# dglai/dgl-0.5-benchmark

Hardware: AMD Instinct MI355X
Metric: aggregated edges/s, full-graph 3-layer GraphSAGE (hidden 64) on an ogbn-products-shaped graph; epoch time in ms_per_step (higher is better)
Workload: dtype f32

## Files before the change

### dgl-0.5-benchmark_amd/csrc/xty.hip

```cpp
#include "common.h"

namespace mgx {

constexpr int kXtyWaves = 2048;

static int xty_waves(int64_t n) {
  int64_t w = (n / 256 + 63) / 64 * 64;
  if (w < 256) w = 256;
  if (w > kXtyWaves) w = kXtyWaves;
  return (int)w;
}

template <int MT, int KT>
__global__ __launch_bounds__(kBlock) void xty_partial_kernel(int64_t n, int M, int K, const float* __restrict__ A, int64_t lda,
                                                             const float* __restrict__ B, int64_t ldb, float* __restrict__ part) {
  const int lane = threadIdx.x & (kWave - 1);
  const int64_t gw = (int64_t)blockIdx.x * kWavesPerBlock + threadIdx.x / kWave;
  const int c = lane % 16, q = lane / 16;
  v4f acc[MT][KT];
#pragma unroll
  for (int i = 0; i < MT; ++i)
#pragma unroll
    for (int j = 0; j < KT; ++j) acc[i][j] = (v4f)(0.f);
  bool am[MT], bm[KT];
// ... 272 lines not shown
  __syncthreads();
  if (sl == 0 && live) {
    float s = 0.f;
    for (int i = 0; i < 16; ++i) s += red[i][e];
    out[(int64_t)(m0 + m) * ldc + k0 + k] = s;
  }
}

template <int MT>
static bool launch_xty_kt(int kt, int waves, int64_t n, int M, int K, const float* A, int64_t lda, const float* B, int64_t ldb,
                          float* part, hipStream_t s) {
  switch (kt) {
#define MGX_XTY(J) case J: hipLaunchKernelGGL((xty_partial_kernel<MT, J>), dim3(waves / kWavesPerBlock), dim3(kBlock), 0, s, n, M, K, A, lda, B, ldb, part); return true;
    MGX_XTY(1) MGX_XTY(2) MGX_XTY(3) MGX_XTY(4) MGX_XTY(5) MGX_XTY(6) MGX_XTY(7) MGX_XTY(8)
#undef MGX_XTY
    default: return false;
  }
}

}

namespace mgx {
__global__ __launch_bounds__(kBlock) void xty_colsum_finish_kernel(int M, int mt16, int waves, const float* __restrict__ part_sum,
                                                                   float* __restrict__ colsum) {
  const int m = blockIdx.x * kWavesPerBlock + threadIdx.x / kWave;
  const int lane = threadIdx.x % kWave;
  if (m >= M) return;
  float s = 0.f;
  for (int w = lane; w < waves; w += kWave) s += part_sum[(int64_t)w * mt16 + m];
#pragma unroll
  for (int off = 32; off >= 1; off >>= 1) s += __shfl_xor(s, off, kWave);
  if (lane == 0) colsum[m] = s;
}
}

extern "C" int64_t mgx_xty_workspace(int64_t M, int64_t K) {
  const int64_t mt = (M + 15) / 16, kt = (K + 15) / 16;
  if (M < 1 || K < 1) return -1;
  if (mt > 4 || kt > 8) {
    if (M > 256 || K > 1024) return -1;
    return (int64_t)mgx::kXtyGridTotal * mgx::kXtyTileM * mgx::kXtyTileK * (int64_t)sizeof(float);
  }
  return (int64_t)mgx::kXtyWaves * (mt * 16 * kt * 16 + mt * 16) * (int64_t)sizeof(float);
}

static int32_t xty_impl(int64_t n, int64_t M, int64_t K, const float* a, int64_t lda, const float* b, int64_t ldb, float* out, int64_t ldc,
                        float* colsum, void* workspace, void* stream, const int64_t* b_rows = nullptr, int mode = 0);

extern "C" int32_t mgx_xty(int64_t n, int64_t M, int64_t K, const float* a, int64_t lda, const float* b, int64_t ldb, float* out,
                           int64_t ldc, void* workspace, void* stream) {
  return xty_impl(n, M, K, a, lda, b, ldb, out, ldc, nullptr, workspace, stream);
}

extern "C" int32_t mgx_xty_colsum(int64_t n, int64_t M, int64_t K, const float* a, int64_t lda, const float* b, int64_t ldb, float* out,
                                  int64_t ldc, float* colsum, void* workspace, void* stream) {
  if (!colsum) return xty_impl(n, M, K, a, lda, b, ldb, out, ldc, nullptr, workspace, stream);
  return xty_impl(n, M, K, a, lda, b, ldb, out, ldc, colsum, workspace, stream);
}

extern "C" int32_t mgx_xty_rows(int64_t n, int64_t M, int64_t K, const float* a, int64_t lda, const float* b, int64_t ldb,
                                const int64_t* b_rows, float* out, int64_t ldc, void* workspace, void* stream) {
  return xty_impl(n, M, K, a, lda, b, ldb, out, ldc, nullptr, workspace, stream, b_rows, b_rows ? mgx::kXtyBRows : 0);
}

extern "C" int32_t mgx_xty_colsum_rows(int64_t n, int64_t M, int64_t K, const float* a, int64_t lda, const float* b, int64_t ldb,
                                       const int64_t* b_rows, float* out, int64_t ldc, float* colsum, void* workspace, void* stream) {
// ... 33 lines not shown
    if (wpt > by_rows) wpt = (int)by_rows;
    if (wpt < 64) wpt = 64;
    hipLaunchKernelGGL(xty_partial_grid_kernel, dim3(wpt / kWavesPerBlock, tiles_m * tiles_k), dim3(kBlock), 0, s, n, (int)M,
                       (int)K, tiles_k, a, lda, b, ldb, part);
    MGX_CHECK_LAUNCH();
    hipLaunchKernelGGL(xty_finish_grid_kernel, dim3(kXtyTileM * kXtyTileK / 16, tiles_m * tiles_k), dim3(kBlock), 0, s, (int)M, (int)K,
                       tiles_k, wpt, (const float*)part, out, ldc);
    MGX_CHECK_LAUNCH();
    return MGX_OK;
  }
  const int waves = xty_waves(n);
  float* part_sum = colsum ? part + (int64_t)kXtyWaves * mt * 16 * kt * 16 : nullptr;
  bool ok = launch_xty_v4(mt, kt, waves, n, (int)M, (int)K, a, lda, b, ldb, part, part_sum, s, b_rows, mode);
  if (!ok && b_rows) MGX_UNSUPPORTED("mgx_xty_rows: no row-list kernel for %lld x %lld", (long long)M, (long long)K);
  if (!ok && colsum) MGX_UNSUPPORTED("mgx_xty_colsum: needs the 16-byte-load form (B: K %% 4 == 0, K >= 64, aligned)");
  if (!ok) switch (mt) {
    case 1: ok = launch_xty_kt<1>(kt, waves, n, (int)M, (int)K, a, lda, b, ldb, part, s); break;
    case 2: ok = launch_xty_kt<2>(kt, waves, n, (int)M, (int)K, a, lda, b, ldb, part, s); break;
    case 3: ok = launch_xty_kt<3>(kt, waves, n, (int)M, (int)K, a, lda, b, ldb, part, s); break;
    default: ok = launch_xty_kt<4>(kt, waves, n, (int)M, (int)K, a, lda, b, ldb, part, s); break;
  }
  MGX_CHECK_ARG(ok, "mgx_xty: no kernel for this tile shape");
  MGX_CHECK_LAUNCH();
  hipLaunchKernelGGL(xty_finish_kernel, dim3((unsigned)((M * K + 15) / 16)), dim3(kBlock), 0, s, (int)M, (int)K, kt * 16,
                     mt * 16 * kt * 16, waves, (const float*)part, out, ldc);
  MGX_CHECK_LAUNCH();
  if (colsum) {
    hipLaunchKernelGGL(xty_colsum_finish_kernel, dim3((unsigned)((M + kWavesPerBlock - 1) / kWavesPerBlock)), dim3(kBlock), 0, s, (int)M,
                       mt * 16, waves, (const float*)part_sum, colsum);
    MGX_CHECK_LAUNCH();
  }
  return MGX_OK;
}
```

### dgl-0.5-benchmark_amd/mi355x_graph/_lib.py

```python
import ctypes
import os

_HERE = os.path.dirname(os.path.abspath(__file__))
CSRC_DIR = os.path.normpath(os.path.join(_HERE, "..", "csrc"))
LIB_PATH = os.environ.get("MGX_LIB_PATH") or os.path.join(CSRC_DIR, "libmi355x_graph.so")
HEADER_PATH = os.path.normpath(os.path.join(_HERE, "..", "..", "include", "mi355x_graph.h"))


class DGLError(RuntimeError):
    """Error type of the DGL operator surface (re-exported as dgl.DGLError)."""


class MgxCsr(ctypes.Structure):
    _fields_ = [
        ("num_rows", ctypes.c_int64),
        ("num_cols", ctypes.c_int64),
        ("nnz", ctypes.c_int64),
        ("indptr", ctypes.c_void_p),
        ("indices", ctypes.c_void_p),
        ("eids", ctypes.c_void_p),
        ("idx_bits", ctypes.c_int32),
        ("reserved", ctypes.c_int32),
    ]

# ... 53 lines not shown
    "mgx_dot_attention_supported": (_i32, [_csr_p, _i64, _i64]),
    "mgx_dot_attention_workspace": (_i64, [_vp, _i64, _i64]),
    "mgx_dot_attention_fwd": (_i32, [_csr_p, _vp, _i64, _i64, _fp, _i64, _fp, _i64, _fp, _i64, ctypes.c_float, _fp, _fp, _vp, _vp]),
    "mgx_dot_attention_bwd": (_i32, [_csr_p, _vp, _csr_p, _vp, _i64, _i64, _fp, _i64, _fp, _i64, _fp, _i64, ctypes.c_float, _fp, _fp, _fp,
                                     _fp, _fp, _fp, _vp, _vp]),
    "mgx_gine_supported": (_i32, [_csr_p, _i64]),
    "mgx_gine_workspace": (_i64, [_vp, _i64]),
    "mgx_gine_fwd": (_i32, [_csr_p, _vp, _i64, _fp, _fp, _fp, _fp, _vp, _vp]),
    "mgx_gine_bwd": (_i32, [_csr_p, _vp, _i64, _fp, _fp, _fp, _fp, _fp, _fp, _vp, _vp]),
    "mgx_head_dot_fwd": (_i32, [_i64, _i64, _i64, _fp, _fp, _fp, _fp, _fp, _vp]),
    "mgx_head_dot_bwd_workspace": (_i64, [_i64, _i64]),
    "mgx_head_dot_bwd": (_i32, [_i64, _i64, _i64, _fp, _fp, _fp, _fp, _fp, _fp, _fp, _fp, _vp, _vp]),
    "mgx_segment_reduce": (_i32, [_i64, _vp, _i64, _i32, _fp, _fp, _vp, _vp]),
    "mgx_segment_softmax_fwd": (_i32, [_i64, _vp, _i64, _fp, _fp, _vp]),
    "mgx_segment_softmax_bwd": (_i32, [_i64, _vp, _i64, _fp, _fp, _fp, _vp]),
    "mgx_segment_attention_supported": (_i32, [_i64, _i64, _i64]),
    "mgx_segment_attention_fwd": (_i32, [_i64, _vp, _i64, _i64, _fp, _i64, _fp, _fp, ctypes.c_float, _fp, _fp, _vp]),
    "mgx_segment_attention_bwd": (_i32, [_i64, _vp, _i64, _i64, _fp, _i64, _fp, _fp, ctypes.c_float, _fp, _fp, _fp, _fp, _fp, _fp, _vp]),
    "mgx_relu_dropout_fwd": (_i32, [_i64, _fp, ctypes.c_float, ctypes.c_uint64, ctypes.c_uint64, _fp, _vp, _vp]),
    "mgx_relu_dropout_bwd": (_i32, [_i64, _fp, _vp, ctypes.c_float, _fp, _vp]),
    "mgx_relu_dropout_fwd_strided": (_i32, [_i64, _i64, _fp, _i64, ctypes.c_float, ctypes.c_uint64, ctypes.c_uint64, _fp, _i64, _vp, _vp]),
    "mgx_relu_dropout_bwd_strided": (_i32, [_i64, _i64, _fp, _i64, _vp, ctypes.c_float, _fp, _i64, _vp]),
    "mgx_relu_dropout_bwd_slots": (_i32, [_i64, _fp, _i64, _vp, ctypes.c_float, _fp, _i64, _fp, _vp, _vp, _vp]),
    "mgx_relu_dropout_fwd_counter": (_i32, [_i64, _i64, _fp, _i64, ctypes.c_float, ctypes.c_uint64, _vp, _fp, _i64, _vp, _vp]),
    "mgx_column_pair_sums": (_i32, [_i64, _i64, _i32, _fp, _fp, _fp, _fp, _vp, _vp]),
    "mgx_column_affine": (_i32, [_i64, _i64, _fp, _fp, _fp, _fp, _fp, _fp, _vp]),
    "mgx_xty_workspace": (_i64, [_i64, _i64]),
    "mgx_xty": (_i32, [_i64, _i64, _i64, _fp, _i64, _fp, _i64, _fp, _i64, _vp, _vp]),
    "mgx_xty_colsum": (_i32, [_i64, _i64, _i64, _fp, _i64, _fp, _i64, _fp, _i64, _fp, _vp, _vp]),
    "mgx_rows_gemm": (_i32, [_i64, _i64, _i64, _fp, _i64, _fp, _i64, _i32, _fp, _fp, _i64, _fp, _i64, _fp, _i64, _i64, _vp]),
    "mgx_xty_rows": (_i32, [_i64, _i64, _i64, _fp, _i64, _fp, _i64, _vp, _fp, _i64, _vp, _vp]),
    "mgx_xty_colsum_rows": (_i32, [_i64, _i64, _i64, _fp, _i64, _fp, _i64, _vp, _fp, _i64, _fp, _vp, _vp]),
    "mgx_xty_colsum_pos": (_i32, [_i64, _i64, _i64, _fp, _i64, _vp, _fp, _i64, _fp, _i64, _fp, _vp, _vp]),
    "mgx_rows_gemm_rows": (_i32, [_i64, _i64, _i64, _fp, _i64, _vp, _fp, _i64, _i32, _fp, _fp, _i64, _fp, _i64, _fp, _i64, _i64, _vp, _vp]),
    "mgx_rows_gemm_supported": (_i32, [_i64, _i64, _i64]),
    "mgx_rows_gemm_sweep_rows": (_i64, [_i64, _i64, _i64, _i32]),
    "mgx_rows_gemm_relu_dropout": (_i32, [_i64, _i64, _i64, _fp, _i64, _fp, _i64, _i32, _fp, ctypes.c_float, ctypes.c_uint64, ctypes.c_uint64,
                                          _fp, _i64, _vp, _vp, _vp, _vp]),
    "mgx_column_sum_workspace": (_i64, [_i64]),
    "mgx_column_sum": (_i32, [_i64, _i64, _fp, _fp, _vp, _vp]),
    "mgx_coo_to_csr_workspace": (_i64, [_i64, _i64, _i32]),
    "mgx_coo_to_csr": (_i32, [_i64, _i64, _vp, _vp, _i32, _vp, _vp, _vp, _vp, _i64, _vp]),
    "mgx_csr_transpose_workspace": (_i64, [_i64, _i64, _i32]),
    "mgx_csr_transpose": (_i32, [_csr_p, _vp, _vp, _vp, _vp, _i64, _vp]),
    "mgx_csr_degrees": (_i32, [_i64, _vp, _i32, _vp, _vp]),
    "mgx_csr_inv_degrees": (_i32, [_i64, _vp, _i32, _fp, _vp]),
    "mgx_coo_to_csr_host": (_i32, [_i64, _i64, _vp, _vp, _i32, _vp, _vp, _vp]),
    "mgx_sample_neighbors": (_i32, [_csr_p, _i64, _vp, _i32, ctypes.c_uint64, _vp, _vp, _vp, _vp]),
    "mgx_sample_count_positive": (_i32, [_csr_p, _i64, _vp, _fp, _vp, _vp, _vp]),
    "mgx_sample_neighbors_weighted": (_i32, [_csr_p, _i64, _vp, _i32, _fp, _i32, ctypes.c_uint64, _vp, _vp, _vp, _vp]),
    "mgx_select_topk": (_i32, [_csr_p, _i64, _vp, _i32, _fp, _i32, _vp, _vp, _vp, _vp]),
    "mgx_to_block_workspace": (_i64, [_i64, _i64]),
    "mgx_to_block": (_i32, [_i64, _i64, _vp, _i64, _vp, _vp, _i32, _i32, _vp, _vp, _vp, _vp, _vp, _vp, _vp]),
    "mgx_node_subgraph_workspace": (_i64, [_i64]),
    "mgx_node_subgraph_count": (_i32, [_csr_p, _i64, _vp, _vp, _vp, _vp, _vp]),
    "mgx_node_subgraph_fill": (_i32, [_csr_p, _i64, _vp, _vp, _vp, _i32, _vp, _vp, _vp, _vp]),
    "mgx_gather_rows": (_i32, [_i64, _vp, _i32, _i64, _fp, _fp, _vp]),
    "mgx_gather_rows_strided": (_i32, [_i64, _vp, _i32, _i64, _fp, _i64, _fp, _i64, _vp]),
    "mgx_scatter_add_rows": (_i32, [_i64, _vp, _i32, _i64, _fp, _fp, _vp]),
}

_lib = None


def lib():
    global _lib
# ... 22 lines not shown
```

### dgl-0.5-benchmark_amd/mi355x_graph/config.py

```python

SAGE_FUSED_LAYER = True
SAGE_CAT = True
SAGE_STATIC_CAT = True
SAGE_FUSED_ADD = True
SAGE_FUSED_ACT = True
SAGE_PROJECT_FIRST = True
SAGE_HEAD_ROWS = True
SAGE_HEAD_INIT = True
ROWS_GEMM = True
LINEAR_XTY = True
XTY_COLSUM = True

GAT_AGG_FIRST = True
GAT_PACK = True

DOT_ATTENTION_FUSED = True
GINE_FUSED = True

SEGMENT_ATTENTION_FUSED = True

DEVICE_BLOCKS = True
DEVICE_SUBGRAPH = True

PLAN_BUILDER = "device"
HUB_SPLIT = 256
LP_ROUNDS = 8
CLUSTER_MIN_NNZ = 4_000_000
TILE_HUB_SPLIT = 2048
TILE_CONFIG = {4: (7, 6, 1, 3), 3: (7, 3, 1, 3), 2: (7, 3, 1, 2)}
GAT_TILE_CONFIG = (7, 3, 1, 2)
TILE_MIN_WIDTH = 4
TILE_VALIDATE = True
SHORT_ROWS_IMBALANCE = 6.0

SPARSE_GRAD = False
SPARSE_GRAD_MIN_NNZ = 2_000_000
WIDE_PAD = True
WIDE_PAD_MIN_NNZ = 1 << 20

PACKED_GATHER = True
PACKED_GATHER_MIN_NNZ = 20_000_000
PACKED_GATHER_PROBE = True
PACKED_GATHER_MAX_OVERFLOW = 0.10

# ... 3 lines not shown
```

### dgl-0.5-benchmark_amd/mi355x_graph/dist.py

```python
import os

import torch
from torch.autograd.function import once_differentiable
import torch.distributed as dist
import torch.nn as nn

from ._lib import DGLError
from . import core, emulate, ops, schedule, sparse
from . import config
from . import function as fn
from .graph import DGLGraph, Frame, GraphIndex


def partition_nodes(src, dst, num_nodes, num_parts, rounds=5, clusters=None):
    dev = src.device
    if num_parts == 1:
        return torch.zeros(num_nodes, dtype=torch.int64, device=dev), {"edge_cut": 0.0, "num_clusters": 1}
    indeg = torch.bincount(dst.long(), minlength=num_nodes)
    node_w = indeg + 1
    if clusters is None:
        csc = sparse.coo_to_csr(num_nodes, num_nodes, dst.contiguous(), src.contiguous())
        cap = int(node_w.sum().item()) // (num_parts * 4) + 1
        hist = schedule.label_propagation(csc.indptr, csc.indices, num_nodes, rounds)
        clusters = _cap_clusters(hist, node_w, cap)
# ... 498 lines not shown
        if plan.n_halo:
            be.spmm_copy_u_strided(plan.halo.csc(), "sum", recv, cat.right, accumulate=True, dst_scale=plan.inv_deg)
        ctx.plan, ctx.comm, ctx.cat, ctx.generation = plan, comm, cat, cat.generation
        ctx.halo_x = halo_x
        comm.mark("dense")
        wcat = torch.cat([w_self, w_neigh], dim=1)
        if act is not None:
            p, into = act
            seed = torch.initial_seed() & (2 ** 64 - 1)
            offset = (ops.ReluDropout._calls * 0x9E3779B97F4A7C15) & (2 ** 63 - 1)
            ops.ReluDropout._calls += 1
            out = None if into is None else into.t
            fused = be.rows_gemm_relu_dropout(cat.buf, wcat, True, bias, float(p), seed, offset, out=out)
            y, mask = fused if fused is not None else be.relu_dropout_fwd(ops._rows_linear(be, cat.buf, wcat, bias), float(p), seed, offset, out=out)
            ctx.save_for_backward(w_self, w_neigh, mask)
            ctx.p = float(p)
            return y
        ctx.save_for_backward(w_self, w_neigh)
        ctx.p = None
        return ops._rows_linear(be, cat.buf, wcat, bias)

    @staticmethod
    @once_differentiable
    def backward(ctx, dy):
        from . import ops
        plan, comm, cat = ctx.plan, ctx.comm, ctx.cat
        if cat.generation != ctx.generation:
            raise DGLError("SAGEConv: a later forward pass overwrote the [h | neigh] buffer this backward pass needs")
        be = sparse.backend_for(dy)
        if ctx.p is not None:
            w_self, w_neigh, mask = ctx.saved_tensors
            if not dy.is_contiguous() and not (hasattr(be, "_row_strided") and be._row_strided(dy)):
                dy = dy.contiguous()
            dy = be.relu_dropout_bwd(dy, mask, ctx.p)
        else:
            w_self, w_neigh = ctx.saved_tensors
        dy = dy.contiguous()
        need = ctx.needs_input_grad
        K = cat.K
        dh = None
        if need[3]:
            dh_own, dn = ops._rows_dgrad(be, dy, torch.cat([w_self, w_neigh], dim=1), plan.inv_deg, K)
            halo_x = ctx.halo_x
            g_halo = torch.empty((plan.n_halo, K), dtype=dy.dtype, device=dy.device)
            comm.mark("halo-row gradients")
            if plan.n_halo:
                be.spmm_copy_u_strided(plan.halo.csr(), "sum", dn, g_halo)
            if halo_x is not None:
                comm.mark("pack")
                halo_x.post_back(g_halo)
            else:
                back = torch.empty((plan.send_idx.shape[0], K), dtype=dy.dtype, device=dy.device)
                work = comm.all_to_all_async(back, g_halo, plan.send_splits, plan.recv_splits)
            comm.mark("owned-row reversed aggregation")
            be.spmm_copy_u_strided(plan.loc.csr(), "sum", dn, dh_own, accumulate=True)
        comm.mark("dense (inside the exchange window)")
        dws = dwn = db = None
        if (need[4] or need[5]) and need[6]:
            dw, db = ops._weight_bias_grad(dy, cat.buf)
            dws, dwn = dw[:, :K].contiguous(), dw[:, K:].contiguous()
        elif need[4] or need[5]:
            dw = ops._weight_grad(dy, cat.buf)
            dws, dwn = dw[:, :K].contiguous(), dw[:, K:].contiguous()
        elif need[6]:
            db = be.column_sum(dy)
        if need[3]:
# ... 447 lines not shown
```

### dgl-0.5-benchmark_amd/mi355x_graph/ops.py

```python
import os

import torch
from torch.autograd.function import once_differentiable

from ._lib import DGLError
from . import sparse
from . import config
from .graph import DGLGraph, GraphIndex

__all__ = ["gspmm", "rel_gspmm", "gsddmm", "edge_softmax", "gat_attention", "gat_fused", "dot_attention", "dot_attention_fused", "gine_sum", "gine_sum_fused", "segment_reduce", "segment_softmax", "segment_attention", "segment_attention_fused", "copy_u_sum", "copy_u_mean", "u_mul_e_sum",
           "copy_e_sum", "u_add_v", "u_dot_v"]


def _torch_ops():
    if os.environ.get("MGX_TORCH_OPS", "auto") != "1":
        return None
    from . import torch_ops
    return torch_ops


_NATIVE = None


def _native_ops():
# ... 761 lines not shown
        n = x.shape[0]
        sdy, sdyx = be.column_pair_sums(dy, x, shifted=True)
        sdyxhat = (sdyx - (mean - x[0]) * sdy) * invstd
        A = invstd if weight is None else weight * invstd
        B = -A * invstd * sdyxhat / n
        Cc = -A * sdy / n - B * mean
        dx = be.column_affine(dy, A.contiguous(), Cc.contiguous(), x, B.contiguous()) if ctx.needs_input_grad[0] else None
        dw = sdyxhat if weight is not None and ctx.needs_input_grad[1] else None
        db = sdy if ctx.needs_input_grad[2] else None
        return dx, dw, db, None


def batch_norm_supported(x):
    return (x.dim() == 2 and x.dtype == torch.float32 and x.device.type in sparse._BACKENDS and x.shape[1] % 4 == 0
            and 4 <= x.shape[1] <= sparse.backend_for(x).COLUMN_SUM_MAX and x.shape[0] > 1)


def _weight_grad(dy2, x2):
    be = sparse.backend_for(dy2)
    if (x2.shape[0] >= be.XTY_MIN_ROWS and dy2.shape[1] <= be.XTY_MAX[0] and x2.shape[1] <= be.XTY_MAX[1]
            and config.LINEAR_XTY):
        return be.xty(dy2 if dy2.stride(1) == 1 else dy2.contiguous(), x2 if x2.stride(1) == 1 else x2.contiguous())
    return dy2.t() @ x2


def _weight_bias_grad(dy2, x2):
    be = sparse.backend_for(dy2)
    if (x2.shape[0] >= be.XTY_MIN_ROWS and dy2.shape[1] <= be.XTY_MAX[0] and x2.shape[1] <= be.XTY_MAX[1]
            and config.LINEAR_XTY and config.XTY_COLSUM):
        return be.xty(dy2 if dy2.stride(1) == 1 else dy2.contiguous(), x2 if x2.stride(1) == 1 else x2.contiguous(), colsum=True)
    return _weight_grad(dy2, x2), be.column_sum(dy2 if dy2.is_contiguous() else dy2.contiguous())


class LinearSumFn(torch.autograd.Function):

    @staticmethod
    def forward(ctx, x1, w1, x2, w2, bias):
        ctx.save_for_backward(x1, w1, x2, w2)
        y = torch.nn.functional.linear(x1, w1, bias)
        return y.addmm_(x2, w2.t())

    @staticmethod
    @once_differentiable
    def backward(ctx, dy):
        x1, w1, x2, w2 = ctx.saved_tensors
        dy = dy.contiguous()
        need = ctx.needs_input_grad
        dx1 = dy @ w1 if need[0] else None
        dw1 = _weight_grad(dy, x1) if need[1] else None
        dx2 = dy @ w2 if need[2] else None
        dw2 = _weight_grad(dy, x2) if need[3] else None
        db = sparse.backend_for(dy).column_sum(dy) if need[4] else None
        return dx1, dw1, dx2, dw2, db


def linear_sum(x1, weight1, x2, weight2, bias=None):
    if (x1.dim() != 2 or x2.dim() != 2 or x1.dtype != torch.float32 or x1.device.type not in sparse._BACKENDS
            or not torch.is_grad_enabled() or (bias is not None and weight1.shape[0] > sparse.backend_for(x1).COLUMN_SUM_MAX)):
        return torch.nn.functional.linear(x1, weight1) + torch.nn.functional.linear(x2, weight2, bias)
    return LinearSumFn.apply(x1, weight1, x2, weight2, bias)


class SelectRowsFn(torch.autograd.Function):

    @staticmethod
    def forward(ctx, x, rows):
# ... 118 lines not shown
            made = act[2] if len(act) > 2 else None
            seed = torch.initial_seed() & (2 ** 64 - 1)
            offset = (ReluDropout._calls * 0x9E3779B97F4A7C15) & (2 ** 63 - 1)
            ReluDropout._calls += 1
            wcat = torch.cat([w_self, w_neigh], dim=1)
            fused = be.rows_gemm_relu_dropout(cat.buf, wcat, True, bias, float(p), seed, offset, out=None if into is None else into.t,
                                              slots=None if made is None else made[0], overflow=None if made is None else made[1])
            if fused is not None and made is not None:
                made[2] = True
            if fused is None:
                y, mask = be.relu_dropout_fwd(_rows_linear(be, cat.buf, wcat, bias), float(p), seed, offset,
                                              out=None if into is None else into.t)
            else:
                y, mask = fused
            ctx.save_for_backward(w_self, w_neigh, mask)
            ctx.p = float(p)
            return y
        ctx.save_for_backward(w_self, w_neigh)
        ctx.p = None
        return _rows_linear(be, cat.buf, torch.cat([w_self, w_neigh], dim=1), bias)

    @staticmethod
    @once_differentiable
    def backward(ctx, dy):
        cat = ctx.cat
        if cat.generation != ctx.generation:
            raise DGLError("SAGEConv: a later forward pass overwrote the [h | neigh] buffer this backward pass needs "
                           "(two forwards before one backward); set MGX_SAGE_CAT=0")
        need = ctx.needs_input_grad
        be = sparse.backend_for(dy)
        K = cat.K
        dh = None
        aggregated_first = False
        if ctx.p is not None:
            w_self, w_neigh, mask = ctx.saved_tensors
            if not dy.is_contiguous() and not be._row_strided(dy):
                dy = dy.contiguous()
            gate = None
            if need[2] and dy.dim() == 2 and dy.shape[1] == 64 and K % 4 == 0 and config.ROWS_GEMM and be.rows_gemm_supported(128, K, 128):
                gate = _slot_gate(be, ctx.gidx, ctx.gidx.csr(), dy.shape[0])
                if gate is not None and not gate.allow():
                    gate = None
            if gate is not None:
                dcat = torch.empty((dy.shape[0], 128), dtype=torch.float32, device=dy.device)
                inv = ctx.gidx.csc().inv_degrees()
                if dy.data_ptr() % 16 == 0:
                    dy, slots, overflow = be.relu_dropout_bwd_slots(dy, mask, ctx.p, dcat[:, :64], row_scale=inv)
                else:
                    dy = be.relu_dropout_bwd(dy, mask, ctx.p, out=dcat[:, :64])
                    slots, overflow = be.rows_slots_pack(dy, row_scale=inv)
                gate.watch(overflow, dy.shape[0])
                be.spmm_copy_u_strided(ctx.gidx.csr(), "sum", dy, dcat[:, 64:], slots=slots, src_scale=inv)
                dh = be.rows_gemm(dcat, torch.cat([w_self, w_neigh], dim=0))
                if dh is None:
                    dh = dcat @ torch.cat([w_self, w_neigh], dim=0)
                aggregated_first = True
            else:
                dy = be.relu_dropout_bwd(dy, mask, ctx.p)
        else:
            w_self, w_neigh = ctx.saved_tensors
        if not aggregated_first:
            dy = dy.contiguous()
        if need[2] and not aggregated_first:
            dh, dn = _rows_dgrad(be, dy, torch.cat([w_self, w_neigh], dim=1), ctx.gidx.csc().inv_degrees(), K)
            be.spmm_copy_u_strided(ctx.gidx.csr(), "sum", dn, dh, accumulate=True)
        dws = dwn = db = None
        if (need[3] or need[4]) and need[5]:
            dw, db = _weight_bias_grad(dy, cat.buf)
            dws, dwn = dw[:, :K].contiguous(), dw[:, K:].contiguous()
        elif need[3] or need[4]:
            dw = _weight_grad(dy, cat.buf)
            dws, dwn = dw[:, :K].contiguous(), dw[:, K:].contiguous()
        elif need[5]:
            db = be.column_sum(dy if dy.is_contiguous() else dy.contiguous())
        return None, None, dh, dws, dwn, db, None


_ROW_BITS = {}


def _row_bits(rows, n, be):
    key = (rows.data_ptr(), int(rows.shape[0]), int(n))
    held = _ROW_BITS.get(key)
    if held is None or held[0] is not rows or held[1] != rows._version:
        flag = torch.zeros((n, 4), dtype=torch.float32, device=rows.device)
        flag[rows] = 1.0
        if len(_ROW_BITS) > 8:
            _ROW_BITS.clear()
        held = _ROW_BITS[key] = (rows, rows._version, be.row_nonzero_bits(flag))
    return held[2]


_ROW_INV_DEG = {}
# ... 728 lines not shown
```

### dgl-0.5-benchmark_amd/mi355x_graph/sparse.py

```python
import ctypes
import os
import functools

import numpy as np
import torch

from . import _lib
from ._lib import DGLError, MgxCsr, OP, REDUCE, TARGET
from . import config


PROFILE = None


class timed_call(object):
    __slots__ = ("rec", "dev")

    def __init__(self, dev, **meta):
        self.rec, self.dev = (meta if PROFILE is not None else None), dev

    def __enter__(self):
        if self.rec is not None:
            self.rec["start"] = torch.cuda.Event(enable_timing=True)
            self.rec["end"] = torch.cuda.Event(enable_timing=True)
# ... 1096 lines not shown
        ws = torch.empty(max(L.mgx_xty_workspace(M, K), 4) // 4, dtype=torch.float32, device=dev)
        with torch.cuda.device(dev):
            if colsum:
                st = L.mgx_xty_colsum_rows(n, M, K, _ptr(a2d), max(a2d.stride(0), M), _ptr(b2d), max(b2d.stride(0), K), _ptr(rows),
                                           _ptr(out), out.stride(0), _ptr(sums), _ptr(ws), _stream(dev))
            else:
                st = L.mgx_xty_rows(n, M, K, _ptr(a2d), max(a2d.stride(0), M), _ptr(b2d), max(b2d.stride(0), K), _ptr(rows),
                                    _ptr(out), out.stride(0), _ptr(ws), _stream(dev))
        if st == _lib.ERR_UNSUPPORTED:
            return None
        _lib.check(st)
        return (out, sums) if colsum else out

    def xty_pos(self, a2d, a_pos, b2d, colsum=False):
        dev = self._check_dev(a2d, b2d, a_pos)
        n, K = b2d.shape
        M = a2d.shape[1]
        tm, tk = self.XTY_TILE
        if (a_pos.dtype != torch.int64 or a_pos.shape != (n,) or not a_pos.is_contiguous() or a2d.shape[0] == 0 or M > tm or K > tk or a2d.stride(1) != 1
                or b2d.stride(1) != 1 or a2d.dtype != torch.float32 or b2d.dtype != torch.float32):
            return None
        L = _lib.lib()
        out = torch.empty((M, K), dtype=torch.float32, device=dev)
        sums = torch.empty(M, dtype=torch.float32, device=dev) if colsum else None
        ws = torch.empty(max(L.mgx_xty_workspace(M, K), 4) // 4, dtype=torch.float32, device=dev)
        with torch.cuda.device(dev):
            st = L.mgx_xty_colsum_pos(n, M, K, _ptr(a2d), max(a2d.stride(0), M), _ptr(a_pos), _ptr(b2d), max(b2d.stride(0), K),
                                      _ptr(out), out.stride(0), _ptr(sums), _ptr(ws), _stream(dev))
        if st == _lib.ERR_UNSUPPORTED:
            return None
        _lib.check(st)
        return (out, sums) if colsum else out

    def xty(self, a2d, b2d, colsum=False, rows=None):
        if rows is not None:
            if rows.dtype != torch.int64 or rows.dim() != 1 or rows.shape[0] != a2d.shape[0] or not rows.is_contiguous():
                raise DGLError("xty: rows must be a contiguous int64 vector with one entry per row of a")
            res = self._xty_rows(a2d, b2d, rows, colsum)
            if res is not None:
                return res
            b2d = b2d.index_select(0, rows)
        dev = self._check_dev(a2d, b2d)
        n, M = a2d.shape
        K = b2d.shape[1]
        if M > self.XTY_MAX[0] or K > self.XTY_MAX[1]:
            raise DGLError("mgx_xty: at most %d x %d outputs, got %d x %d" % (self.XTY_MAX + (M, K)))
        out = torch.empty((M, K), dtype=torch.float32, device=dev)
        sums = torch.empty(M, dtype=torch.float32, device=dev) if colsum else None
        have_sums = False
        L = _lib.lib()
        tm, tk = self.XTY_TILE
        ntiles = ((M + tm - 1) // tm) * ((K + tk - 1) // tk)

        def one(a_t, b_t, o_t, ws, want_sums):
            if want_sums:
                st = L.mgx_xty_colsum(n, a_t.shape[1], b_t.shape[1], _ptr(a_t), max(a2d.stride(0), M), _ptr(b_t), max(b2d.stride(0), K),
                                      _ptr(o_t), out.stride(0), _ptr(sums), _ptr(ws), _stream(dev))
                if st != _lib.ERR_UNSUPPORTED:
                    _lib.check(st)
                    return True
            _lib.check(L.mgx_xty(n, a_t.shape[1], b_t.shape[1], _ptr(a_t), max(a2d.stride(0), M), _ptr(b_t), max(b2d.stride(0), K),
                                 _ptr(o_t), out.stride(0), _ptr(ws), _stream(dev)))
            return False

        with torch.cuda.device(dev):
            if ntiles == 1 or ntiles >= 4:
# ... 488 lines not shown
```

### include/mi355x_graph.h

```cpp
#ifndef MI355X_GRAPH_H_
#define MI355X_GRAPH_H_

#include <stdint.h>

#ifdef __cplusplus
extern "C" {
#endif

typedef enum {
  MGX_OK = 0,
  MGX_ERR_INVALID_ARGUMENT = 1,
  MGX_ERR_UNSUPPORTED = 2,
  MGX_ERR_HIP = 3
} mgx_status;

typedef enum {
  MGX_OP_ADD = 0, MGX_OP_SUB = 1, MGX_OP_MUL = 2, MGX_OP_DIV = 3,
  MGX_OP_COPY_LHS = 4, MGX_OP_COPY_RHS = 5, MGX_OP_DOT = 6
} mgx_op;

typedef enum { MGX_REDUCE_SUM = 0, MGX_REDUCE_MAX = 1, MGX_REDUCE_MIN = 2, MGX_REDUCE_MEAN = 3 } mgx_reduce;

enum {
  MGX_SPMM_ACCUMULATE = 1,
// ... 175 lines not shown
int32_t mgx_gine_bwd(const mgx_csr* csr , const mgx_spmm_plan* plan , int64_t D,
                     const float* x, const float* w, const float* scale, const float* d_out ,
                     float* d_x , float* d_w , void* workspace, void* stream);

int32_t mgx_head_dot_fwd(int64_t n, int64_t H, int64_t F, const float* feat, const float* attn_a,
                         const float* attn_b, float* out_a, float* out_b, void* stream);
int64_t mgx_head_dot_bwd_workspace(int64_t H, int64_t F);
int32_t mgx_head_dot_bwd(int64_t n, int64_t H, int64_t F, const float* feat, const float* attn_a,
                         const float* attn_b, const float* d_out_a, const float* d_out_b, float* d_feat,
                         float* d_attn_a, float* d_attn_b, void* workspace, void* stream);

int32_t mgx_segment_reduce(int64_t num_segments, const int64_t* offsets, int64_t D, int32_t reduce,
                           const float* x, float* out, int64_t* arg, void* stream);

int64_t mgx_column_sum_workspace(int64_t C);
int32_t mgx_column_sum(int64_t n, int64_t C, const float* x, float* out, void* workspace, void* stream);

int32_t mgx_column_pair_sums(int64_t n, int64_t C, int32_t mode, const float* a, const float* b, float* out0, float* out1,
                             void* workspace, void* stream);
int32_t mgx_column_affine(int64_t n, int64_t C, const float* a, const float* b, const float* A, const float* B, const float* Cc,
                          float* out, void* stream);

int64_t mgx_xty_workspace(int64_t M, int64_t K);
int32_t mgx_xty(int64_t n, int64_t M, int64_t K, const float* a, int64_t lda, const float* b, int64_t ldb, float* out, int64_t ldc,
                void* workspace, void* stream);
int32_t mgx_xty_colsum(int64_t n, int64_t M, int64_t K, const float* a, int64_t lda, const float* b, int64_t ldb, float* out, int64_t ldc,
                       float* colsum, void* workspace, void* stream);
int32_t mgx_xty_rows(int64_t n, int64_t M, int64_t K, const float* a, int64_t lda, const float* b, int64_t ldb, const int64_t* b_rows,
                     float* out, int64_t ldc, void* workspace, void* stream);
int32_t mgx_xty_colsum_rows(int64_t n, int64_t M, int64_t K, const float* a, int64_t lda, const float* b, int64_t ldb,
                            const int64_t* b_rows, float* out, int64_t ldc, float* colsum, void* workspace, void* stream);
int32_t mgx_xty_colsum_pos(int64_t n, int64_t M, int64_t K, const float* a, int64_t lda, const int64_t* a_pos, const float* b,
                           int64_t ldb, float* out, int64_t ldc, float* colsum, void* workspace, void* stream);

int32_t mgx_rows_gemm(int64_t n, int64_t K, int64_t M, const float* a, int64_t lda, const float* b, int64_t ldb, int32_t b_transposed,
                      const float* bias , const float* row_scale , int64_t scale_from, float* c,
                      int64_t ldc, float* c2 ,
                      int64_t ldc2, int64_t split_col , void* stream);
int32_t mgx_rows_gemm_rows(int64_t n, int64_t K, int64_t M, const float* a, int64_t lda, const int64_t* a_rows, const float* b, int64_t ldb,
                           int32_t b_transposed, const float* bias, const float* row_scale, int64_t scale_from, float* c, int64_t ldc,
                           float* c2, int64_t ldc2, int64_t split_col, const int64_t* c2_rows, void* stream);
int32_t mgx_rows_gemm_supported(int64_t K, int64_t M, int64_t lda);
int64_t mgx_rows_gemm_sweep_rows(int64_t K, int64_t M, int64_t lda, int32_t relu_dropout);
int32_t mgx_rows_gemm_relu_dropout(int64_t n, int64_t K, int64_t M, const float* a, int64_t lda, const float* b, int64_t ldb,
                                   int32_t b_transposed, const float* bias , float p, uint64_t seed, uint64_t offset,
                                   float* y, int64_t ldy, uint8_t* mask, void* slots ,
                                   int64_t* overflow_rows , void* stream);

int32_t mgx_relu_dropout_fwd(int64_t n, const float* x, float p, uint64_t seed, uint64_t offset, float* y, uint8_t* mask,
                             void* stream);
int32_t mgx_relu_dropout_bwd(int64_t n, const float* dy, const uint8_t* mask, float p, float* dx, void* stream);
int32_t mgx_relu_dropout_fwd_strided(int64_t rows, int64_t cols, const float* x, int64_t x_stride, float p, uint64_t seed,
                                     uint64_t offset, float* y, int64_t y_stride, uint8_t* mask, void* stream);
int32_t mgx_relu_dropout_bwd_strided(int64_t rows, int64_t cols, const float* dy, int64_t dy_stride, const uint8_t* mask, float p,
                                     float* dx, int64_t dx_stride, void* stream);
int32_t mgx_relu_dropout_bwd_slots(int64_t rows, const float* dy, int64_t dy_stride, const uint8_t* mask, float p, float* dx,
                                   int64_t dx_stride, const float* row_scale , void* slots ,
                                   int64_t* overflow_rows , void* stream);
int32_t mgx_relu_dropout_fwd_counter(int64_t rows, int64_t cols, const float* x, int64_t x_stride, float p, uint64_t seed,
                                     const uint64_t* counter, float* y, int64_t y_stride, uint8_t* mask, void* stream);

int32_t mgx_segment_softmax_fwd(int64_t num_segments, const int64_t* offsets, int64_t D, const float* x, float* out, void* stream);
int32_t mgx_segment_softmax_bwd(int64_t num_segments, const int64_t* offsets, int64_t D, const float* out, const float* d_out,
                                float* d_x, void* stream);
int32_t mgx_segment_attention_supported(int64_t H, int64_t F, int64_t feat_ld);
int32_t mgx_segment_attention_fwd(int64_t num_segments, const int64_t* offsets, int64_t H, int64_t F, const float* feat,
// ... 65 lines not shown
```

Before: 41.65 billion.

## Fuse relu-dropout backward into the weight-gradient XᵀY with column sum

Adds a masked XᵀY kernel that applies the dropout mask and scale to dy on the fly while computing the weight gradient and bias column sum. This skips the separate relu_dropout_bwd pass and its materialised output when the input gradient is not needed, as in the first layer. It uses MFMA with software-prefetched operands and a combined finish kernel. Only specific K shapes are compiled, and anything else falls back to the old path.

```diff
diff --git a/dgl-0.5-benchmark_amd/csrc/xty.hip b/dgl-0.5-benchmark_amd/csrc/xty.hip
--- a/dgl-0.5-benchmark_amd/csrc/xty.hip
+++ b/dgl-0.5-benchmark_amd/csrc/xty.hip
@@ -328,6 +328,140 @@
   for (int off = 32; off >= 1; off >>= 1) s += __shfl_xor(s, off, kWave);
   if (lane == 0) colsum[m] = s;
 }
+
+template <int VG0, int ST0, int VG1, int ST1>
+__global__ __launch_bounds__(kBlock) void xty_masked_partial_kernel(int64_t n, int K, int waves, const float* __restrict__ dy, int64_t lddy,
+                                                                    const uint8_t* __restrict__ mask, float scale,
+                                                                    const float* __restrict__ B, int64_t ldb, float* __restrict__ part,
+                                                                    float* __restrict__ part_sum) {
+  constexpr int NG = VG0 + VG1, NS = ST0 + ST1, BT = NG * 4 + NS;
+  constexpr int kDword0 = VG0 * 64, kDword1 = 128 + VG1 * 64;
+  const int lane = threadIdx.x & (kWave - 1);
+  const int wave = __builtin_amdgcn_readfirstlane(threadIdx.x / kWave);
+  const int h = wave & 1;
+  const int64_t gw = (int64_t)blockIdx.x * (kWavesPerBlock / 2) + (wave >> 1);
+  const int c = lane % 16, q = lane / 16;
+  v4f acc[2][BT];
+  v4f accs[2];
+#pragma unroll
+  for (int i = 0; i < 2; ++i) {
+    accs[i] = (v4f)(0.f);
+#pragma unroll
+    for (int j = 0; j < BT; ++j) acc[i][j] = (v4f)(0.f);
+  }
+  const float one = c == 0 ? 1.f : 0.f;
+  const int64_t stride = (int64_t)waves * 16;
+  v2f ra[4];
+  uint32_t rm[4];
+  v4f rg[4][NG > 0 ? NG : 1];
+  float rs[4][NS > 0 ? NS : 1];
+  auto fetch = [&](int64_t r0, int s) {
+    const int64_t row = r0 + s * 4 + q;
+    const int64_t rc = row < n ? row : n - 1;
+    ra[s] = *reinterpret_cast<const v2f*>(dy + rc * lddy + 4 * c + 2 * h);
+    rm[s] = mask[rc * 16 + c];
+    const float* b = B + rc * ldb;
+#pragma unroll
+    for (int g = 0; g < NG; ++g) rg[s][g] = *reinterpret_cast<const v4f*>(b + (g < VG0 ? g * 64 : 128 + (g - VG0) * 64) + 4 * c);
+#pragma unroll
+    for (int t = 0; t < NS; ++t) {
+      const int col = (t < ST0 ? kDword0 + t * 16 : kDword1 + (t - ST0) * 16) + c;
+      rs[s][t] = b[col < K ? col : K - 1];
+    }
+    asm volatile("" ::: "memory");
+  };
+  if (gw * 16 < n) {
+#pragma unroll
+    for (int s = 0; s < 4; ++s) fetch(gw * 16, s);
+  }
+  for (int64_t r0 = gw * 16; r0 < n; r0 += stride) {
+#pragma unroll
+    for (int s = 0; s < 4; ++s) {
+      const bool ok = r0 + s * 4 + q < n;
+      const uint32_t m = ok ? rm[s] >> (2 * h) : 0u;
+      float a[2];
+      a[0] = (m & 1) ? ra[s].x * scale : 0.f;
+      a[1] = (m & 2) ? ra[s].y * scale : 0.f;
+      float b[BT];
+#pragma unroll
+      for (int g = 0; g < NG; ++g) {
+        const v4f v = ok ? rg[s][g] : (v4f)(0.f);
+        b[g * 4 + 0] = v.x; b[g * 4 + 1] = v.y; b[g * 4 + 2] = v.z; b[g * 4 + 3] = v.w;
+      }
+#pragma unroll
+      for (int t = 0; t < NS; ++t) {
+        const int col = (t < ST0 ? kDword0 + t * 16 : kDword1 + (t - ST0) * 16) + c;
+        b[NG * 4 + t] = (ok & (col < K)) ? rs[s][t] : 0.f;
+      }
+#pragma unroll
+      for (int i = 0; i < 2; ++i)
+#pragma unroll
+        for (int j = 0; j < BT; ++j) acc[i][j] = __builtin_amdgcn_mfma_f32_16x16x4f32(a[i], b[j], acc[i][j], 0, 0, 0);
+      const float ones = ok ? one : 0.f;
+#pragma unroll
+      for (int i = 0; i < 2; ++i) accs[i] = __builtin_amdgcn_mfma_f32_16x16x4f32(a[i], ones, accs[i], 0, 0, 0);
+      __builtin_amdgcn_sched_barrier(0);
+      fetch(r0 + stride, s);
+      __builtin_amdgcn_sched_barrier(0);
+    }
+  }
+  float* p = part + gw * (int64_t)64 * K;
+#pragma unroll
+  for (int i = 0; i < 2; ++i)
+#pragma unroll
+    for (int r = 0; r < 4; ++r) {
+      const int mrow = 4 * (4 * q + r) + 2 * h + i;
+      if (c == 0) part_sum[gw * 64 + mrow] = accs[i][r];
+#pragma unroll
+      for (int j = 0; j < BT; ++j) {
+        int k;
+        if (j < NG * 4) {
+          const int g = j / 4;
+          k = (g < VG0 ? g * 64 : 128 + (g - VG0) * 64) + 4 * c + (j % 4);
+        } else {
+          const int t = j - NG * 4;
+          k = (t < ST0 ? kDword0 + t * 16 : kDword1 + (t - ST0) * 16) + c;
+        }
+        if (k < K) p[mrow * K + k] = acc[i][j][r];
+      }
+    }
+}
+
+__global__ __launch_bounds__(kBlock) void xty_masked_finish_kernel(int K, int waves, const float* __restrict__ part,
+                                                                   const float* __restrict__ part_sum, float* __restrict__ out, int64_t ldc,
+                                                                   float* __restrict__ colsum) {
+  __shared__ float red[16][17];
+  const int elem_blocks = 64 * K / 16;
+  if ((int)blockIdx.x >= elem_blocks) {
+    const int m = ((int)blockIdx.x - elem_blocks) * kWavesPerBlock + threadIdx.x / kWave;
+    const int lane = threadIdx.x % kWave;
+    float s = 0.f;
+    for (int w = lane; w < waves; w += kWave) s += part_sum[(int64_t)w * 64 + m];
+#pragma unroll
+    for (int off = 32; off >= 1; off >>= 1) s += __shfl_xor(s, off, kWave);
+    if (lane == 0) colsum[m] = s;
+    return;
+  }
+  const int e = threadIdx.x % 16, sl = threadIdx.x / 16;
+  const int idx = blockIdx.x * 16 + e;
+  const int tile = 64 * K;
+  const float* p = part + idx;
+  const int per = waves / 16;
+  float s0 = 0.f, s1 = 0.f, s2 = 0.f, s3 = 0.f;
+  for (int w = sl * per; w < (sl + 1) * per; w += 4) {
+    s0 += p[(int64_t)w * tile];
+    s1 += p[(int64_t)(w + 1) * tile];
+    s2 += p[(int64_t)(w + 2) * tile];
+    s3 += p[(int64_t)(w + 3) * tile];
+  }
+  red[sl][e] = (s0 + s1) + (s2 + s3);
+  __syncthreads();
+  if (sl == 0) {
+    float s = 0.f;
+    for (int i = 0; i < 16; ++i) s += red[i][e];
+    out[(int64_t)(idx / K) * ldc + idx % K] = s;
+  }
+}
 }
 
 extern "C" int64_t mgx_xty_workspace(int64_t M, int64_t K) {
@@ -427,3 +561,52 @@
   }
   return MGX_OK;
 }
+
+extern "C" int64_t mgx_xty_masked_workspace(int64_t K) {
+  if (K < 64 || K > 256 || K % 4) return -1;
+  return (int64_t)mgx::kXtyWaves * (64 * K + 64) * (int64_t)sizeof(float);
+}
+
+extern "C" int32_t mgx_xty_colsum_masked(int64_t n, int64_t K, const float* dy, int64_t lddy, const uint8_t* mask, float p, const float* b,
+                                         int64_t ldb, float* out, int64_t ldc, float* colsum, void* workspace, void* stream) {
+  using namespace mgx;
+  MGX_ENTER();
+  MGX_CHECK_ARG(n >= 0 && K >= 1, "mgx_xty_colsum_masked: bad sizes");
+  MGX_CHECK_ARG(p >= 0.f && p < 1.f, "mgx_xty_colsum_masked: p must be in [0, 1)");
+  if (K < 64 || K > 256 || K % 4) MGX_UNSUPPORTED("mgx_xty_colsum_masked: needs 64 <= K <= 256, K %% 4 == 0 (got %lld)", (long long)K);
+  MGX_CHECK_ARG(out && colsum, "mgx_xty_colsum_masked: out or colsum is NULL");
+  MGX_CHECK_ARG(lddy >= 64 && ldb >= K && ldc >= K, "mgx_xty_colsum_masked: leading dimensions smaller than the tile (lddy %lld, ldb %lld, ldc %lld)",
+                (long long)lddy, (long long)ldb, (long long)ldc);
+  hipStream_t s = (hipStream_t)stream;
+  if (n == 0) {
+    MGX_CHECK_HIP(hipMemset2DAsync(out, (size_t)ldc * sizeof(float), 0, (size_t)K * sizeof(float), 64, s));
+    MGX_CHECK_HIP(hipMemsetAsync(colsum, 0, 64 * sizeof(float), s));
+    return MGX_OK;
+  }
+  MGX_CHECK_ARG(dy && mask && b && workspace, "mgx_xty_colsum_masked: NULL pointer");
+  if (lddy % 4 || (uintptr_t)dy % 16 || ldb % 4 || (uintptr_t)b % 16)
+    MGX_UNSUPPORTED("mgx_xty_colsum_masked: needs the 16-byte-load form of both operands (row strides %% 4 == 0, 16-byte aligned)");
+  const int64_t k0 = K < 128 ? K : 128, k1 = K - k0;
+  if (k1 > 0 && k1 < 64) MGX_UNSUPPORTED("mgx_xty_colsum_masked: a second block of %lld columns has no 16-byte-load form", (long long)k1);
+  const int vg0 = k0 >= 128 ? 2 : 1, st0 = (int)((k0 - vg0 * 64 + 15) / 16);
+  const int vg1 = k1 >= 128 ? 2 : k1 >= 64 ? 1 : 0, st1 = (int)((k1 - vg1 * 64 + 15) / 16);
+  const int waves = xty_waves(n);
+  float* part = (float*)workspace;
+  float* part_sum = part + (int64_t)kXtyWaves * 64 * K;
+  const float scale = 1.f / (1.f - p);
+  bool ok = false;
+#define MGX_XTYM(A, B, C, D)                                                                                                             \
+  if (vg0 == A && st0 == B && vg1 == C && st1 == D) {                                                                                    \
+    hipLaunchKernelGGL((xty_masked_partial_kernel<A, B, C, D>), dim3(waves / (kWavesPerBlock / 2)), dim3(kBlock), 0, s, n, (int)K, waves, \
+                       dy, lddy, mask, scale, b, ldb, part, part_sum);                                                                   \
+    ok = true;                                                                                                                           \
+  }
+  MGX_XTYM(1, 0, 0, 0) MGX_XTYM(1, 1, 0, 0) MGX_XTYM(2, 0, 0, 0) MGX_XTYM(2, 0, 1, 1) MGX_XTYM(2, 0, 2, 0)
+#undef MGX_XTYM
+  if (!ok) MGX_UNSUPPORTED("mgx_xty_colsum_masked: no kernel for K = %lld (built: 64, 68 .. 80, 128, 196 .. 208, 256)", (long long)K);
+  MGX_CHECK_LAUNCH();
+  hipLaunchKernelGGL(xty_masked_finish_kernel, dim3((unsigned)(64 * K / 16 + 64 / kWavesPerBlock)), dim3(kBlock), 0, s, (int)K, waves,
+                     (const float*)part, (const float*)part_sum, out, ldc, colsum);
+  MGX_CHECK_LAUNCH();
+  return MGX_OK;
+}
diff --git a/dgl-0.5-benchmark_amd/mi355x_graph/_lib.py b/dgl-0.5-benchmark_amd/mi355x_graph/_lib.py
--- a/dgl-0.5-benchmark_amd/mi355x_graph/_lib.py
+++ b/dgl-0.5-benchmark_amd/mi355x_graph/_lib.py
@@ -109,6 +109,8 @@
     "mgx_xty_rows": (_i32, [_i64, _i64, _i64, _fp, _i64, _fp, _i64, _vp, _fp, _i64, _vp, _vp]),
     "mgx_xty_colsum_rows": (_i32, [_i64, _i64, _i64, _fp, _i64, _fp, _i64, _vp, _fp, _i64, _fp, _vp, _vp]),
     "mgx_xty_colsum_pos": (_i32, [_i64, _i64, _i64, _fp, _i64, _vp, _fp, _i64, _fp, _i64, _fp, _vp, _vp]),
+    "mgx_xty_masked_workspace": (_i64, [_i64]),
+    "mgx_xty_colsum_masked": (_i32, [_i64, _i64, _fp, _i64, _vp, ctypes.c_float, _fp, _i64, _fp, _i64, _fp, _vp, _vp]),
     "mgx_rows_gemm_rows": (_i32, [_i64, _i64, _i64, _fp, _i64, _vp, _fp, _i64, _i32, _fp, _fp, _i64, _fp, _i64, _fp, _i64, _i64, _vp, _vp]),
     "mgx_rows_gemm_supported": (_i32, [_i64, _i64, _i64]),
     "mgx_rows_gemm_sweep_rows": (_i64, [_i64, _i64, _i64, _i32]),
diff --git a/dgl-0.5-benchmark_amd/mi355x_graph/config.py b/dgl-0.5-benchmark_amd/mi355x_graph/config.py
--- a/dgl-0.5-benchmark_amd/mi355x_graph/config.py
+++ b/dgl-0.5-benchmark_amd/mi355x_graph/config.py
@@ -10,6 +10,7 @@
 ROWS_GEMM = True
 LINEAR_XTY = True
 XTY_COLSUM = True
+XTY_MASKED = True
 
 GAT_AGG_FIRST = True
 GAT_PACK = True
diff --git a/dgl-0.5-benchmark_amd/mi355x_graph/dist.py b/dgl-0.5-benchmark_amd/mi355x_graph/dist.py
--- a/dgl-0.5-benchmark_amd/mi355x_graph/dist.py
+++ b/dgl-0.5-benchmark_amd/mi355x_graph/dist.py
@@ -554,6 +554,16 @@
             w_self, w_neigh, mask = ctx.saved_tensors
             if not dy.is_contiguous() and not (hasattr(be, "_row_strided") and be._row_strided(dy)):
                 dy = dy.contiguous()
+            need = ctx.needs_input_grad
+            masked = None
+            if not need[3] and (need[4] or need[5]) and need[6] and ops._xty_masked_wanted(be, dy, cat.buf):
+                masked = be.xty_masked(dy, mask, ctx.p, cat.buf)
+            if masked is not None:
+                comm.mark("dense (inside the exchange window)")
+                dw, db = masked
+                dws, dwn = dw[:, :cat.K].contiguous(), dw[:, cat.K:].contiguous()
+                comm.mark("dense")
+                return None, None, None, None, dws, dwn, db, None, None, None
             dy = be.relu_dropout_bwd(dy, mask, ctx.p)
         else:
             w_self, w_neigh = ctx.saved_tensors
diff --git a/dgl-0.5-benchmark_amd/mi355x_graph/ops.py b/dgl-0.5-benchmark_amd/mi355x_graph/ops.py
--- a/dgl-0.5-benchmark_amd/mi355x_graph/ops.py
+++ b/dgl-0.5-benchmark_amd/mi355x_graph/ops.py
@@ -817,6 +817,12 @@
     return _weight_grad(dy2, x2), be.column_sum(dy2 if dy2.is_contiguous() else dy2.contiguous())
 
 
+def _xty_masked_wanted(be, dy2, x2):
+    return (config.XTY_MASKED and os.environ.get("MGX_XTY_MASKED", "1") != "0" and hasattr(be, "xty_masked") and dy2.dim() == 2
+            and x2.shape[0] >= be.XTY_MIN_ROWS and dy2.shape[1] <= be.XTY_MAX[0] and x2.shape[1] <= be.XTY_MAX[1]
+            and config.LINEAR_XTY and config.XTY_COLSUM)
+
+
 class LinearSumFn(torch.autograd.Function):
 
     @staticmethod
@@ -1001,6 +1007,7 @@
         K = cat.K
         dh = None
         aggregated_first = False
+        masked = None
         if ctx.p is not None:
             w_self, w_neigh, mask = ctx.saved_tensors
             if not dy.is_contiguous() and not be._row_strided(dy):
@@ -1025,9 +1032,15 @@
                     dh = dcat @ torch.cat([w_self, w_neigh], dim=0)
                 aggregated_first = True
             else:
-                dy = be.relu_dropout_bwd(dy, mask, ctx.p)
+                if not need[2] and (need[3] or need[4]) and need[5] and _xty_masked_wanted(be, dy, cat.buf):
+                    masked = be.xty_masked(dy, mask, ctx.p, cat.buf)
+                if masked is None:
+                    dy = be.relu_dropout_bwd(dy, mask, ctx.p)
         else:
             w_self, w_neigh = ctx.saved_tensors
+        if masked is not None:
+            dw, db = masked
+            return None, None, None, dw[:, :K].contiguous(), dw[:, K:].contiguous(), db, None
         if not aggregated_first:
             dy = dy.contiguous()
         if need[2] and not aggregated_first:
diff --git a/dgl-0.5-benchmark_amd/mi355x_graph/sparse.py b/dgl-0.5-benchmark_amd/mi355x_graph/sparse.py
--- a/dgl-0.5-benchmark_amd/mi355x_graph/sparse.py
+++ b/dgl-0.5-benchmark_amd/mi355x_graph/sparse.py
@@ -1152,6 +1152,27 @@
         _lib.check(st)
         return (out, sums) if colsum else out
 
+    def xty_masked(self, dy, mask, p, b2d):
+        dev = self._check_dev(dy, mask, b2d)
+        if (dy.dim() != 2 or b2d.dim() != 2 or dy.shape[1] != 64 or b2d.shape[0] != dy.shape[0] or dy.dtype != torch.float32
+                or b2d.dtype != torch.float32 or mask.dtype != torch.uint8 or not mask.is_contiguous() or mask.numel() != dy.shape[0] * 16):
+            return None
+        n, K = b2d.shape
+        if (K < 64 or K > 256 or K % 4 or dy.stride(1) != 1 or b2d.stride(1) != 1 or max(dy.stride(0), 64) % 4 or max(b2d.stride(0), K) % 4
+                or dy.data_ptr() % 16 or b2d.data_ptr() % 16):
+            return None
+        L = _lib.lib()
+        out = torch.empty((64, K), dtype=torch.float32, device=dev)
+        sums = torch.empty(64, dtype=torch.float32, device=dev)
+        ws = torch.empty(L.mgx_xty_masked_workspace(K) // 4, dtype=torch.float32, device=dev)
+        with torch.cuda.device(dev):
+            st = L.mgx_xty_colsum_masked(n, K, _ptr(dy), max(dy.stride(0), 64), _ptr(mask), ctypes.c_float(p), _ptr(b2d), max(b2d.stride(0), K),
+                                         _ptr(out), out.stride(0), _ptr(sums), _ptr(ws), _stream(dev))
+        if st == _lib.ERR_UNSUPPORTED:
+            return None
+        _lib.check(st)
+        return out, sums
+
     def xty(self, a2d, b2d, colsum=False, rows=None):
         if rows is not None:
             if rows.dtype != torch.int64 or rows.dim() != 1 or rows.shape[0] != a2d.shape[0] or not rows.is_contiguous():
diff --git a/experiments/exp_xty_masked.py b/experiments/exp_xty_masked.py
--- /dev/null
+++ b/experiments/exp_xty_masked.py
@@ -0,0 +1,80 @@
+import argparse
+import os
+import statistics
+import sys
+
+import torch
+
+ROOT = os.path.dirname(os.path.dirname(os.path.abspath(__file__)))
+sys.path.insert(0, os.path.join(ROOT, "dgl-0.5-benchmark_amd"))
+from mi355x_graph import sparse
+
+
+def timed(fn, reps):
+    out = []
+    for _ in range(reps):
+        a, b = torch.cuda.Event(enable_timing=True), torch.cuda.Event(enable_timing=True)
+        a.record()
+        fn()
+        b.record()
+        b.synchronize()
+        out.append(a.elapsed_time(b))
+    return out
+
+
+def line(name, ts):
+    print("%-46s median %.3f  min %.3f  max %.3f ms  (%d calls)" % (name, statistics.median(ts), min(ts), max(ts), len(ts)))
+    return statistics.median(ts)
+
+
+def main():
+    ap = argparse.ArgumentParser()
+    ap.add_argument("--n", type=int, default=2449029)
+    ap.add_argument("--K", type=int, default=200)
+    ap.add_argument("--rounds", type=int, default=5)
+    ap.add_argument("--reps", type=int, default=10)
+    args = ap.parse_args()
+    dev = torch.device("cuda:0")
+    be = sparse.backend_for(torch.zeros(1, device=dev))
+    gen = torch.Generator(device=dev).manual_seed(1)
+    n, K = args.n, args.K
+    _, mask = be.relu_dropout_fwd(torch.randn(n, 64, device=dev, generator=gen), 0.5, 11, 5)
+    dy = torch.randn(n, 64, device=dev, generator=gen)
+    b = torch.randn(n, K, device=dev, generator=gen)
+
+    def parent():
+        return be.xty(be.relu_dropout_bwd(dy, mask, 0.5), b, colsum=True)
+
+    def elementwise():
+        return be.relu_dropout_bwd(dy, mask, 0.5)
+
+    dz = be.relu_dropout_bwd(dy, mask, 0.5)
+
+    def xty_only():
+        return be.xty(dz, b, colsum=True)
+
+    def child():
+        return be.xty_masked(dy, mask, 0.5, b)
+
+    want, got = parent(), child()
+    assert got is not None, "no masked kernel for K = %d" % K
+    print("n = %d, K = %d; bitwise equal: out %s, colsum %s" % (n, K, torch.equal(want[0], got[0]), torch.equal(want[1], got[1])))
+    for fn in (parent, elementwise, xty_only, child):
+        timed(fn, 3)
+    t = {"parent": [], "elementwise": [], "xty": [], "child": []}
+    for r in range(args.rounds):
+        t["parent"] += timed(parent, args.reps)
+        t["child"] += timed(child, args.reps)
+        t["elementwise"] += timed(elementwise, args.reps)
+        t["xty"] += timed(xty_only, args.reps)
+    p = line("relu_dropout_bwd + xty(colsum) (parent)", t["parent"])
+    e = line("  relu_dropout_bwd alone", t["elementwise"])
+    line("  xty(colsum) alone", t["xty"])
+    c = line("xty_masked (child)", t["child"])
+    print("gain %.3f ms; the elementwise pass alone %.3f ms; criterion (gain >= elementwise): %s" % (p - c, e, p - c >= e))
+    gb = (n * 64 * 4 + n * 16 + n * K * 4) / 1e9
+    print("child: %.2f GB of operands -> %.2f TB/s; %.1f TFLOP/s of fp32 MFMA (2 n 64 (K + 1))" % (gb, gb / c, 2 * n * 64 * (K + 1) / c / 1e9))
+
+
+if __name__ == "__main__":
+    main()
diff --git a/include/mi355x_graph.h b/include/mi355x_graph.h
--- a/include/mi355x_graph.h
+++ b/include/mi355x_graph.h
@@ -231,6 +231,9 @@
                             const int64_t* b_rows, float* out, int64_t ldc, float* colsum, void* workspace, void* stream);
 int32_t mgx_xty_colsum_pos(int64_t n, int64_t M, int64_t K, const float* a, int64_t lda, const int64_t* a_pos, const float* b,
                            int64_t ldb, float* out, int64_t ldc, float* colsum, void* workspace, void* stream);
+int64_t mgx_xty_masked_workspace(int64_t K);
+int32_t mgx_xty_colsum_masked(int64_t n, int64_t K, const float* dy, int64_t lddy, const uint8_t* mask, float p, const float* b,
+                              int64_t ldb, float* out, int64_t ldc, float* colsum, void* workspace, void* stream);
 
 int32_t mgx_rows_gemm(int64_t n, int64_t K, int64_t M, const float* a, int64_t lda, const float* b, int64_t ldb, int32_t b_transposed,
                       const float* bias , const float* row_scale , int64_t scale_from, float* c,
```

Measured after the change: 42.89 billion (median of 6 runs). 3.0% higher.
